# sea-with-sakura/ViT-of-Pytorch

Hardware: AMD Instinct MI355X
Metric: images/sec training step, ViT-B/16 224px bf16, 1/2/4/8 MI355X (higher is better)
Workload: dtype bf16; 1 GPU; ViT-B16 @224 train step (fwd+CE+bwd+SGD-momentum/OneCycleLR); model=ViT-B16, image_size=224, per_gpu_batch=256, global_batch=256, seq_len=197, num_classes=1000, parallelism=dp1, step_launch=eager

## Files before the change

vit-of-pytorch_amd/csrc/gemm.hip:

```cpp
#include "gemm_decl.h"

namespace {
using vitg::GemmDev;
using vitg::EPI_DROP;

int pick_tile(const vit_gemm_args* a) {
  if (a->tile > 0) return (int)a->tile;
  const bool ak = a->a_layout == VIT_K_CONTIG, bk = a->b_layout == VIT_K_CONTIG;
  if (a->epilogue == VIT_EPI_SPLITK && a->M >= 256 && a->N >= 256) {
    static const int env_sk = vit::knob("VIT_GEMM_SPLITK_CFG", 9);
    return env_sk == 5 || env_sk == 6 || env_sk == 7 || env_sk == 8 ? env_sk : 9;
  }
  if (a->M >= 1024 && a->N >= 256) {
    static const int env_rs = vit::knob("VIT_GEMM_RESID_PP2", 1);
    if (ak && (env_rs || !(a->epilogue == VIT_EPI_BIAS_RESID_F32 && a->K < 2048))) return 9;
    if (a->N >= 2048 && a->epilogue != VIT_EPI_GELU_BWD && a->epilogue != VIT_EPI_MUL_BF16) return 5;
    if (!bk && a->K >= 3072) return 5;
    return 3;
  }
  return 0;
}

int tile_rows_of(int cfg) {
  switch (cfg) {
    case 1: case 2: case 3: case 5: case 6: case 7: case 8: case 9: case 10: case 11: return 256;
    default: return 128;
  }
}

long wave_split_rows(const vit_gemm_args* a, int cfg) {
  if (!((cfg == 5 || cfg == 9) && a->batch == 1 && a->split_k == 1 && a->epilogue != VIT_EPI_PATCH && a->tile == 0))
    return 0;
  static const int ncu = [] {
    int dev = 0, n = 0;
    if (hipGetDevice(&dev) != hipSuccess || hipDeviceGetAttribute(&n, hipDeviceAttributeMultiprocessorCount, dev) !=
                                               hipSuccess)
      return 0;
    return n;
  }();
  if (ncu <= 0) return 0;
  const long tiles_n = (a->N + 255) / 256, tiles = ((a->M + 255) / 256) * tiles_n;
  const long full = tiles / ncu, rem = tiles - full * ncu;
  const long main_rows = (full * ncu / tiles_n) * 256;
  return full >= 1 && rem > 0 && 2 * rem <= ncu && main_rows > 0 && main_rows < a->M ? main_rows : 0;
}

int rem_config() {
  static const int rem_cfg = vit::knob("VIT_GEMM_REM_CFG", 0);
  return rem_cfg >= 0 && rem_cfg <= 9 && rem_cfg != 1 ? rem_cfg : 0;
}

}

extern "C" int64_t vit_gemm_tile_rows(const vit_gemm_args* a) {
  if (!a) return 0;
  return tile_rows_of(pick_tile(a));
}

extern "C" int64_t vit_gemm_partial_rows(const vit_gemm_args* a) {
  if (!a) return 0;
  const int cfg = pick_tile(a);
  const long main_rows = wave_split_rows(a, cfg);
  if (main_rows > 0) {
    const long rr = tile_rows_of(rem_config());
    return main_rows / 256 + (a->M - main_rows + rr - 1) / rr;
  }
  const long tr = tile_rows_of(cfg);
  return (a->M + tr - 1) / tr;
}

extern "C" int64_t vit_gemm_split_rows(const vit_gemm_args* a) {
  if (!a) return 0;
  return wave_split_rows(a, pick_tile(a));
}

#ifdef VIT_PP2_STAMPS
static unsigned long long* g_pp2_stamp_buf = nullptr;
extern "C" int vit_gemm_set_stamps(void* dev_buf) {
  g_pp2_stamp_buf = (unsigned long long*)dev_buf;
  return 0;
}
#endif

namespace {
int make_dev(const vit_gemm_args* a, GemmDev& d, bool& empty) {
  empty = false;
  VIT_CHECK_ARG(a != nullptr, "vit_gemm_bf16: null args");
  VIT_CHECK_ARG(a->M >= 0 && a->N >= 0 && a->K >= 0, "vit_gemm_bf16: negative size");
  VIT_CHECK_ARG(a->K % 64 == 0, "vit_gemm_bf16: K=%lld must be a multiple of 64", (long long)a->K);
  VIT_CHECK_ARG(a->M < (1 << 30) && a->N < (1 << 30), "vit_gemm_bf16: M/N too large");
  VIT_CHECK_ARG(a->A && a->B && a->C, "vit_gemm_bf16: null operand");
  VIT_CHECK_ARG(a->batch >= 1 && a->split_k >= 1, "vit_gemm_bf16: batch/split_k must be >= 1");
  VIT_CHECK_ARG(a->split_k == 1 || a->epilogue == VIT_EPI_SPLITK, "vit_gemm_bf16: split_k>1 needs VIT_EPI_SPLITK");
  VIT_CHECK_ARG(a->a_layout == VIT_K_CONTIG || a->a_layout == VIT_MN_CONTIG, "vit_gemm_bf16: bad a_layout");
  VIT_CHECK_ARG(a->b_layout == VIT_K_CONTIG || a->b_layout == VIT_MN_CONTIG, "vit_gemm_bf16: bad b_layout");
  if (a->M == 0 || a->N == 0) {
    empty = true;
    return VIT_OK;
  }
  const bool ak = a->a_layout == VIT_K_CONTIG, bk = a->b_layout == VIT_K_CONTIG;
  const long a_rows = ak ? a->M : a->K, a_cols = ak ? a->K : a->M;
  const long b_rows = bk ? a->N : a->K, b_cols = bk ? a->K : a->N;
  VIT_CHECK_ARG(a->lda >= a_cols && a->ldb >= b_cols, "vit_gemm_bf16: leading dimension too small");
  VIT_CHECK_ARG(a->lda % 8 == 0 && a->ldb % 8 == 0, "vit_gemm_bf16: lda/ldb must be multiples of 8");
  VIT_CHECK_ARG(((uintptr_t)a->A | (uintptr_t)a->B) % 16 == 0 && (a->a_batch_stride | a->b_batch_stride) % 8 == 0,
                "vit_gemm_bf16: A/B must be 16-byte aligned");
  const long a_bytes = ((a_rows - 1) * a->lda + ((a_cols + 7) & ~7L)) * 2;
  const long b_bytes = ((b_rows - 1) * a->ldb + ((b_cols + 7) & ~7L)) * 2;
  VIT_CHECK_ARG(a_bytes < (1L << 31) && b_bytes < (1L << 31), "vit_gemm_bf16: operand larger than 2 GiB");
  switch (a->epilogue) {
    case VIT_EPI_BIAS_GELU: VIT_CHECK_ARG(a->C2 != nullptr, "GELU epilogue needs C2"); break;
    case VIT_EPI_BIAS_RESID_F32: VIT_CHECK_ARG(a->aux != nullptr, "RESID epilogue needs aux"); break;
    case VIT_EPI_GELU_BWD: VIT_CHECK_ARG(a->aux != nullptr, "GELU_BWD epilogue needs aux"); break;
    case VIT_EPI_MUL_BF16: VIT_CHECK_ARG(a->aux != nullptr, "MUL epilogue needs aux"); break;
    case VIT_EPI_BIAS_GELU_DGELU: VIT_CHECK_ARG(a->C2 != nullptr, "GELU_DGELU epilogue needs C2"); break;
    case VIT_EPI_PATCH:
      VIT_CHECK_ARG(a->aux && a->aux2 && a->bias && a->tokens > 0 && a->batch == 1, "PATCH epilogue args");
      break;
    default: break;
  }
  d = GemmDev{};
  d.M = (int)a->M; d.N = (int)a->N; d.K = (int)a->K;
  d.A = (const char*)a->A; d.lda = a->lda; d.a_bs = a->a_batch_stride; d.a_bytes = (uint32_t)a_bytes;
  d.B = (const char*)a->B; d.ldb = a->ldb; d.b_bs = a->b_batch_stride; d.b_bytes = (uint32_t)b_bytes;
  d.C = a->C; d.ldc = a->ldc; d.c_bs = a->c_batch_stride;
  d.C2 = a->C2; d.ldc2 = a->ldc2;
  d.bias = a->bias; d.bias_bs = a->bias_batch_stride;
  d.aux = a->aux; d.ldaux = a->ldaux; d.aux2 = a->aux2;
  d.split_k = (int)a->split_k; d.tokens = (int)a->tokens;
  {
    auto al = [](const void* q) { return ((uintptr_t)q % 32) == 0; };
    bool v = al(a->C) && a->ldc % 8 == 0 && a->c_batch_stride % 8 == 0;
    if (a->C2) v = v && al(a->C2) && a->ldc2 % 8 == 0;
    if (a->bias) v = v && al(a->bias) && a->bias_batch_stride % 8 == 0;
    if (a->aux) v = v && al(a->aux) && a->ldaux % 8 == 0;
    if (a->aux2) v = v && al(a->aux2);
    if (a->epilogue == VIT_EPI_SPLITK) v = al(a->C) && a->N % 8 == 0;
    d.vec = v ? 1 : 0;
  }
  d.col_partial = a->col_partial;
  d.drop = make_drop(a->dropout);
  VIT_CHECK_ARG(!d.drop.thr || a->epilogue == VIT_EPI_PATCH || a->epilogue == VIT_EPI_BIAS_RESID_F32 ||
                    a->epilogue == VIT_EPI_BIAS_GELU_DGELU,
                "vit_gemm_bf16: dropout is supported on the PATCH, BIAS_RESID_F32 and BIAS_GELU_DGELU epilogues");
  VIT_CHECK_ARG(!d.drop.thr || (a->a_layout == VIT_K_CONTIG &&
                                  (a->b_layout == VIT_K_CONTIG || a->epilogue == VIT_EPI_BIAS_RESID_F32)),
                "vit_gemm_bf16: dropout epilogues need a K-contiguous A (and B, except BIAS_RESID_F32)");
  {
    static const int env_gm = vit::knob("VIT_GEMM_GROUP_M", 8);
    static const int env_nt = vit::knob("VIT_GEMM_NT", 0);
    d.group_m = env_gm;
    d.nt = env_nt;
    static const int env_diag = vit::knob("VIT_GEMM_DIAG", 0);
    d.diag = env_diag;
    static const int env_sx = vit::knob("VIT_GEMM_SPLIT_XCD", 1);
    d.split_xcd = env_sx;
    static const int env_prio = vit::knob("VIT_GEMM_PRIO", 1);
    d.prio = env_prio;
    static const int env_ilv = vit::knob("VIT_GEMM_ILV", -1);
    d.ilv = env_ilv;
#ifdef VIT_PP2_STAMPS
    d.stamps = g_pp2_stamp_buf;
#endif
  }
  return VIT_OK;
}

int gemm_bf16_impl(const vit_gemm_args* a, int part, vit_stream_t stream) {
  GemmDev d;
  bool empty = false;
  if (const int rc = make_dev(a, d, empty)) return rc;
  if (empty) return VIT_OK;
  const bool ak = a->a_layout == VIT_K_CONTIG, bk = a->b_layout == VIT_K_CONTIG;
  if (a->col_partial) {
    VIT_CHECK_ARG(a->batch == 1 && a->split_k == 1 && d.vec && a->N % 8 == 0 &&
                      (a->epilogue == VIT_EPI_F32 || a->epilogue == VIT_EPI_BF16 || a->epilogue == VIT_EPI_GELU_BWD ||
                       a->epilogue == VIT_EPI_MUL_BF16 ||
                       a->epilogue == VIT_EPI_BIAS_BF16 || a->epilogue == VIT_EPI_BIAS_RESID_F32),
                  "vit_gemm_bf16: col_partial needs batch 1, split_k 1, aligned N%%8==0 operands and a plain epilogue");
  }
  hipStream_t s = (hipStream_t)stream;
  const int batch = (int)a->batch, split = (int)a->split_k;
  const int cfg = pick_tile(a);
#ifdef VIT_DIAG_KNOBS
  VIT_CHECK_ARG(cfg >= 0 && cfg <= 11, "vit_gemm_bf16: bad tile config %d", cfg);
#else
  VIT_CHECK_ARG(cfg >= 0 && cfg <= 9, "vit_gemm_bf16: bad tile config %d", cfg);
#endif
  VIT_CHECK_ARG(cfg != 1 || a->K % 32 == 0, "vit_gemm_bf16: K");
  auto run = [&](int c, const GemmDev& g) -> hipError_t {
    switch (a->epilogue) {
      case VIT_EPI_F32: return vitg::launch_layout_x<VIT_EPI_F32>(c, g, ak, bk, batch, split, s);
      case VIT_EPI_BF16: return vitg::launch_layout_x<VIT_EPI_BF16>(c, g, ak, bk, batch, split, s);
      case VIT_EPI_BIAS_BF16: return vitg::launch_layout_x<VIT_EPI_BIAS_BF16>(c, g, ak, bk, batch, split, s);
      case VIT_EPI_BIAS_GELU: return vitg::launch_layout_x<VIT_EPI_BIAS_GELU>(c, g, ak, bk, batch, split, s);
      case VIT_EPI_BIAS_RESID_F32:
        if (g.drop.thr) return vitg::launch_kk_x<VIT_EPI_BIAS_RESID_F32 | EPI_DROP>(c, g, bk, batch, split, s);
        return vitg::launch_layout_x<VIT_EPI_BIAS_RESID_F32>(c, g, ak, bk, batch, split, s);
      case VIT_EPI_GELU_BWD: return vitg::launch_layout_x<VIT_EPI_GELU_BWD>(c, g, ak, bk, batch, split, s);
      case VIT_EPI_BIAS_GELU_DGELU:
        if (g.drop.thr) return vitg::launch_kk_x<VIT_EPI_BIAS_GELU_DGELU | EPI_DROP>(c, g, bk, batch, split, s);
        return vitg::launch_layout_x<VIT_EPI_BIAS_GELU_DGELU>(c, g, ak, bk, batch, split, s);
      case VIT_EPI_MUL_BF16: return vitg::launch_layout_x<VIT_EPI_MUL_BF16>(c, g, ak, bk, batch, split, s);
      case VIT_EPI_PATCH:
        if (g.drop.thr) return vitg::launch_kk_x<VIT_EPI_PATCH | EPI_DROP>(c, g, bk, batch, split, s);
        return vitg::launch_layout_x<VIT_EPI_PATCH>(c, g, ak, bk, batch, split, s);
      case VIT_EPI_SPLITK: return vitg::launch_layout_x<VIT_EPI_SPLITK>(c, g, ak, bk, batch, split, s);
      default: return hipErrorInvalidValue;
    }
  };
  if (a->epilogue < 0 || a->epilogue > VIT_EPI_MUL_BF16) {
    vit::set_error("vit_gemm_bf16: unknown epilogue %d", a->epilogue);
    return VIT_ERR_INVALID_ARG;
  }
  if (const long main_rows = wave_split_rows(a, cfg)) {
    GemmDev g1 = d, g2 = d;
    g1.M = (int)main_rows;
    g2.M = (int)(a->M - main_rows);
    const long r0 = main_rows;
    const long a_off = ak ? r0 * a->lda * 2 : r0 * 2;
    g2.A = d.A + a_off;
    g2.a_bytes = d.a_bytes > a_off ? (uint32_t)(d.a_bytes - a_off) : 0u;
    const int csz = (a->epilogue == VIT_EPI_F32 || a->epilogue == VIT_EPI_BIAS_RESID_F32) ? 4 : 2;
    g2.C = (char*)d.C + r0 * a->ldc * csz;
    if (d.C2) g2.C2 = (char*)d.C2 + r0 * a->ldc2 * 2;
    if (d.aux) g2.aux = (const char*)d.aux + r0 * a->ldaux * (a->epilogue == VIT_EPI_BIAS_RESID_F32 ? 4 : 2);
    if (d.col_partial) g2.col_partial = d.col_partial + (main_rows / 256) * a->N;
    g2.drop.row0 = (int)r0;
    hipError_t e = hipSuccess;
    if (part != 2) e = run(cfg, g1);
    if (e == hipSuccess && part != 1) e = run(rem_config(), g2);
    return vit::check_hip(e, "vit_gemm_bf16 launch");
  }
  if (part == 2) return VIT_OK;
  return vit::check_hip(run(cfg, d), "vit_gemm_bf16 launch");
}
}

extern "C" int vit_gemm_bf16(const vit_gemm_args* a, vit_stream_t stream) { return gemm_bf16_impl(a, 0, stream); }

extern "C" int vit_gemm_bf16_part(const vit_gemm_args* a, int32_t part, vit_stream_t stream) {
  VIT_CHECK_ARG(part == 1 || part == 2, "vit_gemm_bf16_part: part %d (1 = whole-wave rows, 2 = remainder)", part);
  return gemm_bf16_impl(a, part, stream);
}

extern "C" int vit_gemm_splitk_group(const vit_gemm_args* args, int32_t n, vit_stream_t stream) {
  VIT_CHECK_ARG(args != nullptr && n >= 1 && n <= vitg::GEMM_GROUP_MAX, "vit_gemm_splitk_group: 1..%d members, got %d",
                vitg::GEMM_GROUP_MAX, n);
  vitg::GemmGroup g{};
  long total = 0;
  for (int i = 0; i < n; ++i) {
    const vit_gemm_args* a = args + i;
    VIT_CHECK_ARG(a->epilogue == VIT_EPI_SPLITK && a->a_layout == VIT_MN_CONTIG && a->b_layout == VIT_MN_CONTIG &&
                      a->tile == 0 && !a->col_partial && !a->dropout,
                  "vit_gemm_splitk_group: member %d must be a split-K weight gradient (VIT_EPI_SPLITK, both operands "
                  "M/N-contiguous, no tile / col_partial / dropout)", i);
    bool empty = false;
    if (const int rc = make_dev(a, g.g[i], empty)) return rc;
    VIT_CHECK_ARG(!empty, "vit_gemm_splitk_group: member %d is empty", i);
    g.start[i] = (int)total;
    total += ((a->M + 255) / 256) * ((a->N + 255) / 256) * a->split_k * a->batch;
    VIT_CHECK_ARG(total < (1L << 30), "vit_gemm_splitk_group: grid too large");
  }
  g.start[n] = (int)total;
  g.n = n;
  return vit::check_hip(vitg::launch_splitk_group(g, (hipStream_t)stream), "vit_gemm_splitk_group launch");
}

namespace {
__global__ void splitk_reduce_kernel(const float* __restrict__ ws, int split, long M, long N, float* __restrict__ out,
                                     long ldo, long obs, int accumulate) {
  const int z = blockIdx.y;
  const long total = M * N;
  const float* w = ws + (long)z * split * total;
  float* o = out + z * obs;
  for (long i = (long)blockIdx.x * blockDim.x + threadIdx.x; i < total; i += (long)gridDim.x * blockDim.x) {
    float s = 0.f;
    for (int k = 0; k < split; ++k) s += w[k * total + i];
    const long m = i / N, n = i - m * N;
    float* dst = o + m * ldo + n;
    *dst = accumulate ? *dst + s : s;
  }
}
__global__ void splitk_reduce4_kernel(const float* __restrict__ ws, int split, long M, long N, float* __restrict__ out,
                                      long ldo, long obs, int accumulate) {
  const int z = blockIdx.y;
  const long total = M * N, total4 = total / 4;
  const float4* w = reinterpret_cast<const float4*>(ws + (long)z * split * total);
  float* o = out + z * obs;
  for (long i = (long)blockIdx.x * blockDim.x + threadIdx.x; i < total4; i += (long)gridDim.x * blockDim.x) {
    float4 s = make_float4(0.f, 0.f, 0.f, 0.f);
    int k = 0;
    for (; k + 4 <= split; k += 4) {
      const float4 a = w[(long)k * total4 + i], b = w[(long)(k + 1) * total4 + i];
      const float4 c = w[(long)(k + 2) * total4 + i], d = w[(long)(k + 3) * total4 + i];
      s.x += (a.x + b.x) + (c.x + d.x);
      s.y += (a.y + b.y) + (c.y + d.y);
      s.z += (a.z + b.z) + (c.z + d.z);
      s.w += (a.w + b.w) + (c.w + d.w);
    }
    for (; k < split; ++k) {
      const float4 a = w[(long)k * total4 + i];
      s.x += a.x; s.y += a.y; s.z += a.z; s.w += a.w;
    }
    const long e = i * 4, m = e / N, n = e - m * N;
    float4* dst = reinterpret_cast<float4*>(o + m * ldo + n);
    if (accumulate) {
      const float4 p = *dst;
      s.x += p.x; s.y += p.y; s.z += p.z; s.w += p.w;
    }
    *dst = s;
  }
}

struct SplitkJobDev {
  const float* ws;
  float* out;
  long M, N, ldo, obs;
  int split, batch, nb, blk0, acc;
};
struct SplitkGroupDev {
  SplitkJobDev j[VIT_SPLITK_GROUP_MAX];
  int n;
};
__global__ void splitk_reduce4_group_kernel(const SplitkGroupDev G) {
  int jx = 0;
#pragma unroll
  for (int k = 1; k < VIT_SPLITK_GROUP_MAX; ++k)
    if (k < G.n && (int)blockIdx.x >= G.j[k].blk0) jx = k;
  const SplitkJobDev& J = G.j[jx];
  const int local = blockIdx.x - J.blk0;
  const int z = local / J.nb, bx = local - z * J.nb;
  const long total = J.M * J.N, total4 = total / 4;
  const float4* w = reinterpret_cast<const float4*>(J.ws + (long)z * J.split * total);
  float* o = J.out + z * J.obs;
  for (long i = (long)bx * blockDim.x + threadIdx.x; i < total4; i += (long)J.nb * blockDim.x) {
    float4 s = make_float4(0.f, 0.f, 0.f, 0.f);
    int k = 0;
    for (; k + 4 <= J.split; k += 4) {
      const float4 a = w[(long)k * total4 + i], b = w[(long)(k + 1) * total4 + i];
      const float4 c = w[(long)(k + 2) * total4 + i], d = w[(long)(k + 3) * total4 + i];
      s.x += (a.x + b.x) + (c.x + d.x);
      s.y += (a.y + b.y) + (c.y + d.y);
      s.z += (a.z + b.z) + (c.z + d.z);
      s.w += (a.w + b.w) + (c.w + d.w);
    }
    for (; k < J.split; ++k) {
      const float4 a = w[(long)k * total4 + i];
      s.x += a.x; s.y += a.y; s.z += a.z; s.w += a.w;
    }
    const long e = i * 4, m = e / J.N, n = e - m * J.N;
    float4* dst = reinterpret_cast<float4*>(o + m * J.ldo + n);
    if (J.acc) {
      const float4 p = *dst;
      s.x += p.x; s.y += p.y; s.z += p.z; s.w += p.w;
    }
    *dst = s;
  }
}
}

extern "C" int vit_splitk_reduce_group(const vit_splitk_job* jobs, int32_t n, vit_stream_t stream) {
  VIT_CHECK_ARG(jobs && n >= 1 && n <= VIT_SPLITK_GROUP_MAX, "vit_splitk_reduce_group: 1..%d jobs, got %d",
                VIT_SPLITK_GROUP_MAX, (int)n);
  bool vec = true;
  for (int k = 0; k < n; ++k) {
    const vit_splitk_job& j = jobs[k];
    VIT_CHECK_ARG(j.ws && j.out && j.batch >= 1 && j.split >= 1 && j.M >= 1 && j.N >= 1 && j.ldo >= j.N,
                  "vit_splitk_reduce_group: job %d: bad args", k);
    vec = vec && j.N % 4 == 0 && j.ldo % 4 == 0 && j.out_batch_stride % 4 == 0 && ((uintptr_t)j.ws % 16) == 0 &&
          ((uintptr_t)j.out % 16) == 0;
  }
  if (!vec) {
    for (int k = 0; k < n; ++k) {
      const vit_splitk_job& j = jobs[k];
      if (const int rc = vit_splitk_reduce(j.ws, j.batch, j.split, j.M, j.N, j.out, j.ldo, j.out_batch_stride,
                                           j.accumulate, stream))
        return rc;
    }
    return VIT_OK;
  }
  SplitkGroupDev g{};
  long blk = 0;
  for (int k = 0; k < n; ++k) {
    const vit_splitk_job& j = jobs[k];
    long nb = (j.M * j.N / 4 + 255) / 256;
    if (nb > 4096) nb = 4096;
    SplitkJobDev& d = g.j[k];
    d.ws = j.ws; d.out = j.out; d.M = j.M; d.N = j.N; d.ldo = j.ldo; d.obs = j.out_batch_stride;
    d.split = (int)j.split; d.batch = (int)j.batch; d.nb = (int)nb; d.blk0 = (int)blk; d.acc = j.accumulate ? 1 : 0;
    blk += nb * j.batch;
  }
  g.n = n;
  VIT_CHECK_ARG(blk < (1L << 31), "vit_splitk_reduce_group: grid too large");
  hipLaunchKernelGGL(splitk_reduce4_group_kernel, dim3((unsigned)blk), dim3(256), 0, (hipStream_t)stream, g);
  VIT_LAUNCH_CHECK("vit_splitk_reduce_group");
}

extern "C" int vit_splitk_reduce(const float* ws, int64_t batch, int64_t split, int64_t M, int64_t N, float* out,
                                 int64_t ldo, int64_t out_batch_stride, int32_t accumulate, vit_stream_t stream) {
  VIT_CHECK_ARG(ws && out && batch >= 1 && split >= 1 && ldo >= N, "vit_splitk_reduce: bad args");
  if (M * N == 0) return VIT_OK;
  const bool vec = N % 4 == 0 && ldo % 4 == 0 && out_batch_stride % 4 == 0 && ((uintptr_t)ws % 16) == 0 &&
                   ((uintptr_t)out % 16) == 0;
  long blocks = (M * N / (vec ? 4 : 1) + 255) / 256;
  if (blocks > 4096) blocks = 4096;
  if (vec)
    hipLaunchKernelGGL(splitk_reduce4_kernel, dim3((unsigned)blocks, (unsigned)batch), dim3(256), 0,
                       (hipStream_t)stream, ws, (int)split, (long)M, (long)N, out, (long)ldo, (long)out_batch_stride,
                       (int)accumulate);
  else
    hipLaunchKernelGGL(splitk_reduce_kernel, dim3((unsigned)blocks, (unsigned)batch), dim3(256), 0, (hipStream_t)stream,
                       ws, (int)split, (long)M, (long)N, out, (long)ldo, (long)out_batch_stride, (int)accumulate);
  VIT_LAUNCH_CHECK("vit_splitk_reduce");
}
```

vit-of-pytorch_amd/csrc/gemm_decl.h:

```cpp
#pragma once
#include "common.h"
#include <stdlib.h>

namespace vitg {

struct GemmDev {
  int M, N, K;
  const char* A;
  long lda;
  long a_bs;
  uint32_t a_bytes;
  const char* B;
  long ldb;
  long b_bs;
  uint32_t b_bytes;
  void* C;
  long ldc;
  long c_bs;
  void* C2;
  long ldc2;
  const float* bias;
  long bias_bs;
  const void* aux;
  long ldaux;
  const float* aux2;
  int split_k;
  int tokens;
  int vec;
  float* col_partial;
  int group_m;
  int nt;
  DropDev drop;
  int diag;
  int split_xcd;
  int prio;
  int ilv;
#ifdef VIT_PP2_STAMPS
  unsigned long long* stamps;
#endif
};

constexpr int GEMM_GROUP_MAX = 4;
struct GemmGroup {
  GemmDev g[GEMM_GROUP_MAX];
  int start[GEMM_GROUP_MAX + 1];
  int n;
};
hipError_t launch_splitk_group(const GemmGroup& g, hipStream_t s);

constexpr int EPI_DROP = 16;

template <int EPI>
hipError_t launch_layout_x(int cfg, const GemmDev& d, bool ak, bool bk, int batch, int split, hipStream_t s);
template <int EPI>
hipError_t launch_kk_x(int cfg, const GemmDev& d, bool bk, int batch, int split, hipStream_t s);
template <> hipError_t launch_layout_x<0>(int, const GemmDev&, bool, bool, int, int, hipStream_t);
template <> hipError_t launch_layout_x<1>(int, const GemmDev&, bool, bool, int, int, hipStream_t);
template <> hipError_t launch_layout_x<2>(int, const GemmDev&, bool, bool, int, int, hipStream_t);
template <> hipError_t launch_layout_x<3>(int, const GemmDev&, bool, bool, int, int, hipStream_t);
template <> hipError_t launch_layout_x<4>(int, const GemmDev&, bool, bool, int, int, hipStream_t);
template <> hipError_t launch_layout_x<5>(int, const GemmDev&, bool, bool, int, int, hipStream_t);
template <> hipError_t launch_layout_x<6>(int, const GemmDev&, bool, bool, int, int, hipStream_t);
template <> hipError_t launch_layout_x<7>(int, const GemmDev&, bool, bool, int, int, hipStream_t);
template <> hipError_t launch_layout_x<8>(int, const GemmDev&, bool, bool, int, int, hipStream_t);
template <> hipError_t launch_layout_x<9>(int, const GemmDev&, bool, bool, int, int, hipStream_t);
template <> hipError_t launch_kk_x<20>(int, const GemmDev&, bool, int, int, hipStream_t);
template <> hipError_t launch_kk_x<22>(int, const GemmDev&, bool, int, int, hipStream_t);
template <> hipError_t launch_kk_x<24>(int, const GemmDev&, bool, int, int, hipStream_t);
}
```

vit-of-pytorch_amd/csrc/gemm_pp2.inc:

```
template <bool AK, bool BKC, int EPI, int BK = 64, int NA = 2>
__device__ __forceinline__ void pp2_tile(const GemmDev& p, const int tm, const int tn, const int z,
                                         const int split_idx, const int orig) {
  constexpr int BM = 256, BN = 256, KK = BK / 32;
  constexpr int NB = NA + 1;
  constexpr int TN = BN / 4, FM = 8, FN = TN / 16;
  constexpr int HALF = 128 * BK * 2;
  constexpr int A0_OFF = 0, A1_OFF = NA * HALF, B_OFF = 2 * NA * HALF;
  constexpr int LDS = (2 * NA + 2 * NB) * HALF;
  constexpr int I = BK / 16;
  constexpr int LDW = TN + 4;
  constexpr int PR = 32;
  constexpr int WST = PR * LDW * 4;
  static_assert(8 * WST <= LDS && LDS <= 160 * 1024, "LDS budget / epilogue staging");
  static_assert(2 * I * (NA - 1) <= 32 && (2 * NA - 1) * I <= 62 && 2 * (NB - 1) * I <= 62, "vmcnt range");
  __shared__ __attribute__((aligned(16))) char smem[LDS];

  const int lane = threadIdx.x & 63;
  const int wave = __builtin_amdgcn_readfirstlane(threadIdx.x >> 6);
  const int grp = wave >> 2, wn = wave & 3;
  const int m0 = tm * BM, n0 = tn * BN;
  if (p.diag >= 100 && ((orig >> 3) & 1) && (orig >> 3) < 32) {
    const unsigned long long t0 = __builtin_amdgcn_s_memrealtime();
    while (__builtin_amdgcn_s_memrealtime() - t0 < (unsigned long long)(p.diag - 100) * 100ull)
      __builtin_amdgcn_s_sleep(8);
  }

  const char* Ab = p.A + (long)z * p.a_bs * 2;
  const char* Bb = p.B + (long)z * p.b_bs * 2;
  const long a_shift = AK ? (long)m0 * p.lda * 2 : (long)m0 * 2;
  const long b_shift = BKC ? (long)n0 * p.ldb * 2 : (long)n0 * 2;
  const uint32_t a_rec = (long)p.a_bytes > a_shift ? (uint32_t)(p.a_bytes - a_shift) : 0u;
  const uint32_t b_rec = (long)p.b_bytes > b_shift ? (uint32_t)(p.b_bytes - b_shift) : 0u;
  const __amdgpu_buffer_rsrc_t rsA = make_rsrc(Ab + a_shift, a_rec);
  const __amdgpu_buffer_rsrc_t rsB = make_rsrc(Bb + b_shift, b_rec);
  const int a_h1 = AK ? (int)(128 * p.lda * 2) : 256;
  const int b_h1 = BKC ? (int)(128 * p.ldb * 2) : 256;

  const int nkt = p.K / BK;
  const int kt0 = (int)((long)nkt * split_idx / p.split_k);
  const int kt1 = (int)((long)nkt * (split_idx + 1) / p.split_k);
  const int nk = kt1 - kt0;

  v4f acc[FM][FN];
#pragma unroll
  for (int i = 0; i < FM; ++i)
#pragma unroll
    for (int j = 0; j < FN; ++j) acc[i][j] = v4f{0.f, 0.f, 0.f, 0.f};
  v8s af[KK][FM], bfr[KK][FN];
  const int w4 = wave & 3;
#ifdef VIT_PP2_STAMPS
  const bool stw = p.diag == 4 && p.stamps && orig == 0 && split_idx == 0 && z == 0 && w4 == 0;
  unsigned long long stv[8] = {0, 0, 0, 0, 0, 0, 0, 0};
#define PP2_ST(k)                                          \
  do {                                                     \
    if (stw && j == nk / 2) {                              \
      __builtin_amdgcn_sched_barrier(0);                   \
      stv[k] = __builtin_amdgcn_s_memtime();               \
      __builtin_amdgcn_sched_barrier(0);                   \
    }                                                      \
  } while (0)
#else
#define PP2_ST(k) \
  do {            \
  } while (0)
#endif

  auto ld_a = [&](int h, int t) {
    stage_tile<128, BK, AK, 4>(smem, (h ? A1_OFF : A0_OFF) + (t % NA) * HALF, rsA, p.lda, kt0 + t, w4, lane,
                               h ? a_h1 : 0);
  };
  auto ld_b = [&](int h, int t) {
    stage_tile<128, BK, BKC, 4>(smem, B_OFF + (t % NB) * 2 * HALF + h * HALF, rsB, p.ldb, kt0 + t, w4, lane,
                                h ? b_h1 : 0);
  };
  uint32_t a_lane[AK ? 1 : FM], b_lane[BKC ? 1 : FN];
  if constexpr (!AK) {
#pragma unroll
    for (int i = 0; i < FM; ++i) a_lane[i] = frag_tr_lane_off<128>(i * 16, lane);
  }
  if constexpr (!BKC) {
#pragma unroll
    for (int jn = 0; jn < FN; ++jn) b_lane[jn] = frag_tr_lane_off<128>((wn & 1) * 64 + jn * 16, lane);
  }
  const uint32_t s0 = (uint32_t)(uintptr_t)LDS_PTR(char, smem);
  auto mem = [&](int t) {
    const int aoff = (grp ? A1_OFF : A0_OFF) + (t % NA) * HALF;
    const int boff = B_OFF + (t % NB) * 2 * HALF + (wn >> 1) * HALF;
    const uint32_t ab = __builtin_amdgcn_readfirstlane(s0 + aoff), bb = __builtin_amdgcn_readfirstlane(s0 + boff);
#pragma unroll
    for (int kk = 0; kk < KK; ++kk) {
#pragma unroll
      for (int jn = 0; jn < FN; ++jn) {
        if constexpr (BKC)
          bfr[kk][jn] = read_frag<128, BK, BKC>(smem, boff, (wn & 1) * 64 + jn * 16, kk, lane);
        else
          bfr[kk][jn] = kk == 0 ? read_frag_tr_asm<128, 0>(b_lane[jn] + bb) : read_frag_tr_asm<128, 1>(b_lane[jn] + bb);
      }
#pragma unroll
      for (int i = 0; i < FM; ++i) {
        if constexpr (AK)
          af[kk][i] = read_frag<128, BK, AK>(smem, aoff, i * 16, kk, lane);
        else
          af[kk][i] = kk == 0 ? read_frag_tr_asm<128, 0>(a_lane[i] + ab) : read_frag_tr_asm<128, 1>(a_lane[i] + ab);
      }
    }
  };
#ifdef VIT_DIAG_KNOBS
  const bool ilv = p.ilv < 0 ? (!AK && !BKC) : p.ilv > 0;
#else
  constexpr bool ilv = !AK && !BKC;
#endif
  auto frag = [&](int t, int f) {
    constexpr int NF = FN + FM;
    const int kk = f / NF, r = f % NF;
    const int aoff = (grp ? A1_OFF : A0_OFF) + (t % NA) * HALF;
    const int boff = B_OFF + (t % NB) * 2 * HALF + (wn >> 1) * HALF;
    const uint32_t ab = __builtin_amdgcn_readfirstlane(s0 + aoff), bb = __builtin_amdgcn_readfirstlane(s0 + boff);
    if (r < FN) {
      if constexpr (BKC)
        bfr[kk][r] = read_frag<128, BK, BKC>(smem, boff, (wn & 1) * 64 + r * 16, kk, lane);
      else
        bfr[kk][r] = kk == 0 ? read_frag_tr_asm<128, 0>(b_lane[r] + bb) : read_frag_tr_asm<128, 1>(b_lane[r] + bb);
    } else {
      const int i = r - FN;
      if constexpr (AK)
        af[kk][i] = read_frag<128, BK, AK>(smem, aoff, i * 16, kk, lane);
      else
        af[kk][i] = kk == 0 ? read_frag_tr_asm<128, 0>(a_lane[i] + ab) : read_frag_tr_asm<128, 1>(a_lane[i] + ab);
    }
  };
  auto piece = [&](int q, int j, bool g1) {
    __builtin_amdgcn_sched_barrier(0);
    if (q < I) {
      const int t = g1 ? j + NA : j + NA - 1;
      if (t < nk)
        stage_piece<128, BK, AK, 4>(smem, (g1 ? A0_OFF : A1_OFF) + (t % NA) * HALF, rsA, p.lda, kt0 + t, w4, lane,
                                    g1 ? 0 : a_h1, q);
    } else {
      const int t = j + NB - 1;
      if (t < nk)
        stage_piece<128, BK, BKC, 4>(smem, B_OFF + (t % NB) * 2 * HALF + (g1 ? HALF : 0), rsB, p.ldb, kt0 + t, w4,
                                     lane, g1 ? b_h1 : 0, q - I);
    }
    __builtin_amdgcn_sched_barrier(0);
  };
  auto slot_ilv = [&](int j, bool g1) {
    constexpr int NFR = KK * (FN + FM), NP = 2 * I, PER = NFR / NP;
    static_assert(PER * NP == NFR, "whole fragments between pieces");
#pragma unroll
    for (int f = 0; f < NFR; ++f) {
      frag(j, f);
      if (f % PER == PER - 1) piece(f / PER, j, g1);
    }
  };
  auto reads_done = [&]() {
    asm volatile("s_waitcnt lgkmcnt(0)" ::: "memory");
    __builtin_amdgcn_sched_barrier(0);
  };
  auto compute = [&]() {
    if (p.prio == 1) __builtin_amdgcn_s_setprio(1);
#pragma unroll
    for (int kk = 0; kk < KK; ++kk)
#pragma unroll
      for (int i = 0; i < FM; ++i)
#pragma unroll
        for (int jn = 0; jn < FN; ++jn)
          acc[i][jn] = __builtin_amdgcn_mfma_f32_16x16x32_bf16(__builtin_bit_cast(v8bf, af[kk][i]),
                                                               __builtin_bit_cast(v8bf, bfr[kk][jn]), acc[i][jn], 0, 0, 0);
    if (p.prio == 1) __builtin_amdgcn_s_setprio(0);
  };
  auto read_prio = [&](bool hi) {
    if (p.prio == 2) {
      if (hi) __builtin_amdgcn_s_setprio(1);
      else __builtin_amdgcn_s_setprio(0);
    }
  };
  auto barrier = [&]() {
    __builtin_amdgcn_sched_barrier(0);
    asm volatile("s_barrier" ::: "memory");
    __builtin_amdgcn_sched_barrier(0);
  };
  auto wait_younger = [&](int younger) {
    __builtin_amdgcn_sched_barrier(0);
    if constexpr (NA == 2 && I == 4) {
      if (younger >= 8)
        wait_vm<8>();
      else if (younger >= 4)
        wait_vm<4>();
      else
        wait_vm<0>();
    } else {
      switch (younger / I) {
        case 0: wait_vm<0>(); break;
        case 1: wait_vm<I>(); break;
        case 2: wait_vm<2 * I>(); break;
        case 3: wait_vm<3 * I>(); break;
        case 4: wait_vm<4 * I>(); break;
        case 5: wait_vm<5 * I>(); break;
        case 6: wait_vm<6 * I>(); break;
        case 7: wait_vm<7 * I>(); break;
        default: wait_vm<8 * I>(); break;
      }
    }
  };
  auto dma0 = [&](int j) { return j < 0 ? 0 : I * ((j + NA - 1 < nk) + (j + NB - 1 < nk)); };
  auto dma1 = [&](int j) { return j < 0 ? 0 : I * ((j + NA < nk) + (j + NB - 1 < nk)); };
  auto in_flight = [&](int j, bool g1) {
    int n = 0;
#pragma unroll
    for (int d = 0; d < NA - 1; ++d) n += g1 ? dma1(j - d) : dma0(j - d);
    return n;
  };

  if (grp == 0) {
#pragma unroll
    for (int t = 0; t < NA; ++t)
      if (t < nk) ld_a(0, t);
#pragma unroll
    for (int t = 0; t < NA - 1; ++t)
      if (t < nk) ld_a(1, t);
  } else {
#pragma unroll
    for (int t = 0; t < NB - 1; ++t)
      if (t < nk) {
        ld_b(0, t);
        ld_b(1, t);
      }
  }
  wait_vm<0>();
  __builtin_amdgcn_s_barrier();
  asm volatile("" ::: "memory");

  if (grp == 0) {
    for (int j = 0; j < nk; ++j) {
      PP2_ST(0);
      read_prio(true);
      if (ilv) {
        slot_ilv(j, false);
        PP2_ST(1);
      } else {
        mem(j);
        PP2_ST(1);
        if (j + NA - 1 < nk) ld_a(1, j + NA - 1);
        if (j + NB - 1 < nk) ld_b(0, j + NB - 1);
      }
      read_prio(false);
      PP2_ST(2);
      reads_done();
      PP2_ST(3);
      wait_younger(in_flight(j, false));
      PP2_ST(4);
      barrier();
      PP2_ST(5);
      compute();
      PP2_ST(6);
      barrier();
      PP2_ST(7);
    }
  } else if (nk > 0) {
    barrier();
    for (int j = 0; j < nk; ++j) {
      PP2_ST(0);
      read_prio(true);
      if (ilv) {
        slot_ilv(j, true);
        PP2_ST(1);
      } else {
        mem(j);
        PP2_ST(1);
        if (j + NA < nk) ld_a(0, j + NA);
        if (j + NB - 1 < nk) ld_b(1, j + NB - 1);
      }
      read_prio(false);
      PP2_ST(2);
      reads_done();
      PP2_ST(3);
      wait_younger(in_flight(j, true));
      PP2_ST(4);
      barrier();
      PP2_ST(5);
      compute();
      PP2_ST(6);
      if (j + 1 < nk) barrier();
      PP2_ST(7);
    }
  }
#ifdef VIT_PP2_STAMPS
  if (stw && lane == 0) {
#pragma unroll
    for (int k = 0; k < 8; ++k) p.stamps[grp * 8 + k] = stv[k];
  }
#endif
#undef PP2_ST

  if (p.diag == 2) {
    float t = 0.f;
#pragma unroll
    for (int i = 0; i < FM; ++i)
#pragma unroll
      for (int jn = 0; jn < FN; ++jn) t += acc[i][jn][0] + acc[i][jn][1] + acc[i][jn][2] + acc[i][jn][3];
    if (t == 1234.5f) ((float*)p.C)[threadIdx.x] = t;
    return;
  }
  const int wm0 = grp * 128, wn0 = wn * TN;
  const int g = lane >> 4, c = lane & 15;
  float* ws = reinterpret_cast<float*>(smem + wave * WST);
  constexpr int CPR = TN / 8;
  float csum[8] = {0.f, 0.f, 0.f, 0.f, 0.f, 0.f, 0.f, 0.f};
  constexpr int IT = PR * CPR / 64;
  static_assert(IT * 64 == PR * CPR, "whole chunks per pass");
  constexpr int AW = AuxPre<EPI>::W > 0 ? AuxPre<EPI>::W : 1;
  uint4 axc[IT][AW], axn[IT][AW];
  auto fetch_pass = [&](uint4 (*ax)[AW], int pass) {
    if constexpr (AuxPre<EPI>::W > 0) {
#pragma unroll
      for (int it = 0; it < IT; ++it) {
        const int e = lane + it * 64, row = e / CPR, ch = e % CPR;
        const int m = m0 + wm0 + pass * PR + row, n = n0 + wn0 + ch * 8;
        if (p.vec && m < p.M && n + 8 <= p.N) AuxPre<EPI>::fetch(p, m, n, ax[it]);
      }
    }
  };
  if (EpiOut<EPI>::FAST && p.vec && p.diag == 0 && m0 + BM <= p.M && n0 + BN <= p.N) {
    epilogue_fast<EPI, FN, LDW, CPR>(p, acc, ws, lane, m0 + wm0, n0 + wn0, z, split_idx, csum);
  } else {
  fetch_pass(axc, 0);
#pragma unroll
  for (int pass = 0; pass < 128 / PR; ++pass) {
    if (pass + 1 < 128 / PR) fetch_pass(axn, pass + 1);
#pragma unroll
    for (int i = 0; i < PR / 16; ++i)
#pragma unroll
      for (int jn = 0; jn < FN; ++jn)
#pragma unroll
        for (int r = 0; r < 4; ++r) ws[(i * 16 + 4 * g + r) * LDW + jn * 16 + c] = acc[pass * (PR / 16) + i][jn][r];
    asm volatile("s_waitcnt lgkmcnt(0)" ::: "memory");
    __builtin_amdgcn_wave_barrier();
#pragma unroll
    for (int it = 0; it < IT; ++it) {
      const int e = lane + it * 64, row = e / CPR, ch = e % CPR;
      const int m = m0 + wm0 + pass * PR + row, n = n0 + wn0 + ch * 8;
      float v[8];
      ld8f(ws + row * LDW + ch * 8, v);
      if (m >= p.M || n >= p.N || p.diag == 1 || (p.diag == 3 && (blockIdx.x & 1))) continue;
      if (p.vec && n + 8 <= p.N) {
        if constexpr (AuxPre<EPI>::W > 0) {
          float u[8];
          AuxPre<EPI>::unpack(axc[it], u);
          epi_store8<EPI>(p, z, split_idx, m, n, v, u);
        } else {
          epi_store8<EPI>(p, z, split_idx, m, n, v);
        }
        if (p.col_partial) {
#pragma unroll
          for (int k = 0; k < 8; ++k) csum[k] += v[k];
        }
      } else {
#pragma unroll
        for (int k = 0; k < 8; ++k) epi_store<EPI>(p, z, split_idx, m, n + k, v[k]);
      }
    }
    asm volatile("s_waitcnt lgkmcnt(0)" ::: "memory");
    __builtin_amdgcn_wave_barrier();
    if constexpr (AuxPre<EPI>::W > 0) {
#pragma unroll
      for (int it = 0; it < IT; ++it)
#pragma unroll
        for (int w = 0; w < AW; ++w) axc[it][w] = axn[it][w];
    }
  }
  }
  if (p.col_partial) {
#pragma unroll
    for (int k = 0; k < 8; ++k)
#pragma unroll
      for (int o = CPR; o < 64; o <<= 1) csum[k] += __shfl_xor(csum[k], o, 64);
    __syncthreads();
    float* red = reinterpret_cast<float*>(smem);
    if (lane < CPR) {
#pragma unroll
      for (int k = 0; k < 8; ++k) red[grp * BN + wn0 + lane * 8 + k] = csum[k];
    }
    __syncthreads();
    for (int col = threadIdx.x; col < BN; col += 512)
      if (n0 + col < p.N) p.col_partial[(long)tm * p.N + n0 + col] = red[col] + red[BN + col];
  }
}

__device__ __forceinline__ void splitk_coords(const GemmDev& p, int w, int nwg, int tiles_m, int tiles_n, int& tm, int& tn,
                                              int& z, int& split_idx) {
  const int zs = w / nwg;
  z = zs / p.split_k;
  split_idx = zs % p.split_k;
  tile_coords(w % nwg, tiles_m, tiles_n, p.group_m, tm, tn);
}

__device__ __forceinline__ int xcd_major(int lin, int total) {
  const int xcd = lin & 7, q8 = total >> 3, r8 = total & 7;
  return (xcd < r8 ? xcd * (q8 + 1) : r8 * (q8 + 1) + (xcd - r8) * q8) + (lin >> 3);
}

template <bool AK, bool BKC, int EPI, int BK = 64, int NA = 2>
__global__ void __launch_bounds__(512) gemm_pp2_kernel(const GemmDev p) {
  const int tiles_m = (p.M + 255) / 256, tiles_n = (p.N + 255) / 256;
  const int nwg = tiles_m * tiles_n;
  const int orig = blockIdx.x;
  int tm, tn, z, split_idx;
  if (p.split_k > 1 && p.split_xcd) {
    const int total = nwg * p.split_k * (int)gridDim.z;
    const int lin = blockIdx.x + nwg * (blockIdx.y + p.split_k * blockIdx.z);
    splitk_coords(p, xcd_major(lin, total), nwg, tiles_m, tiles_n, tm, tn, z, split_idx);
  } else {
    tile_coords(xcd_major(orig, nwg), tiles_m, tiles_n, p.group_m, tm, tn);
    z = blockIdx.z;
    split_idx = blockIdx.y;
  }
  pp2_tile<AK, BKC, EPI, BK, NA>(p, tm, tn, z, split_idx, orig);
}

template <bool AK, bool BKC>
__global__ void __launch_bounds__(512) gemm_pp2_group_kernel(const GemmGroup G) {
  const int orig = blockIdx.x;
  const int w = xcd_major(orig, G.start[G.n]);
  int gi = 0;
#pragma unroll
  for (int k = 1; k < GEMM_GROUP_MAX; ++k)
    if (k < G.n && w >= G.start[k]) gi = k;
  gi = __builtin_amdgcn_readfirstlane(gi);
  const GemmDev& p = G.g[gi];
  const int tiles_m = (p.M + 255) / 256, tiles_n = (p.N + 255) / 256;
  int tm, tn, z, split_idx;
  splitk_coords(p, w - G.start[gi], tiles_m * tiles_n, tiles_m, tiles_n, tm, tn, z, split_idx);
  pp2_tile<AK, BKC, VIT_EPI_SPLITK>(p, tm, tn, z, split_idx, orig);
}

template <bool AK, bool BKC, int EPI, int BK = 64, int NA = 2>
hipError_t launch_pp2(const GemmDev& d, int batch, int split, hipStream_t s) {
  const int tiles = ((d.M + 255) / 256) * ((d.N + 255) / 256);
  dim3 grid(tiles, split, batch);
  hipLaunchKernelGGL((gemm_pp2_kernel<AK, BKC, EPI, BK, NA>), grid, dim3(512), 0, s, d);
  return hipGetLastError();
}

inline hipError_t launch_pp2_group(const GemmGroup& g, hipStream_t s) {
  hipLaunchKernelGGL((gemm_pp2_group_kernel<false, false>), dim3(g.start[g.n]), dim3(512), 0, s, g);
  return hipGetLastError();
}
```

Before: 7769 images/sec.

## Let each wave group load its own A half in the MN-contig pp2 GEMM

For the pp2 256x256 GEMM tile with both operands non-K-contiguous, each wave group now issues the global-to-LDS load of its own A half right after its compute phase. Before, the loads were spread across the two groups' interleaved fragment-read slots. The counted vmcnt waits are rewritten to match the new per-group in-flight load counts, and B loads stay interleaved with the fragment reads. The aim is to cut cross-group dependencies and put A prefetch under compute. The risk is a wrong wait count, which would race on LDS, and a different issue balance that can stall the memory pipe.

```diff
diff --git a/vit-of-pytorch_amd/csrc/gemm.hip b/vit-of-pytorch_amd/csrc/gemm.hip
--- a/vit-of-pytorch_amd/csrc/gemm.hip
+++ b/vit-of-pytorch_amd/csrc/gemm.hip
@@ -159,6 +159,8 @@
     d.prio = env_prio;
     static const int env_ilv = vit::knob("VIT_GEMM_ILV", -1);
     d.ilv = env_ilv;
+    static const int env_own = vit::knob("VIT_GEMM_OWN", 1);
+    d.own = env_own;
 #ifdef VIT_PP2_STAMPS
     d.stamps = g_pp2_stamp_buf;
 #endif
diff --git a/vit-of-pytorch_amd/csrc/gemm_decl.h b/vit-of-pytorch_amd/csrc/gemm_decl.h
--- a/vit-of-pytorch_amd/csrc/gemm_decl.h
+++ b/vit-of-pytorch_amd/csrc/gemm_decl.h
@@ -35,6 +35,7 @@
   int split_xcd;
   int prio;
   int ilv;
+  int own;
 #ifdef VIT_PP2_STAMPS
   unsigned long long* stamps;
 #endif
diff --git a/vit-of-pytorch_amd/csrc/gemm_pp2.inc b/vit-of-pytorch_amd/csrc/gemm_pp2.inc
--- a/vit-of-pytorch_amd/csrc/gemm_pp2.inc
+++ b/vit-of-pytorch_amd/csrc/gemm_pp2.inc
@@ -13,6 +13,8 @@
   constexpr int WST = PR * LDW * 4;
   static_assert(8 * WST <= LDS && LDS <= 160 * 1024, "LDS budget / epilogue staging");
   static_assert(2 * I * (NA - 1) <= 32 && (2 * NA - 1) * I <= 62 && 2 * (NB - 1) * I <= 62, "vmcnt range");
+  constexpr int OWN_PIECES = (!AK && !BKC && NA == 2) ? I : 0;
+  static_assert(OWN_PIECES == 0 || OWN_PIECES == I, "whole A halves move; the counted waits below assume it");
   __shared__ __attribute__((aligned(16))) char smem[LDS];
 
   const int lane = threadIdx.x & 63;
@@ -50,7 +52,7 @@
   const int w4 = wave & 3;
 #ifdef VIT_PP2_STAMPS
   const bool stw = p.diag == 4 && p.stamps && orig == 0 && split_idx == 0 && z == 0 && w4 == 0;
-  unsigned long long stv[8] = {0, 0, 0, 0, 0, 0, 0, 0};
+  unsigned long long stv[10] = {0, 0, 0, 0, 0, 0, 0, 0, 0, 0};
 #define PP2_ST(k)                                          \
   do {                                                     \
     if (stw && j == nk / 2) {                              \
@@ -106,8 +108,10 @@
     }
   };
 #ifdef VIT_DIAG_KNOBS
+  const bool own = OWN_PIECES > 0 && p.own != 0;
   const bool ilv = p.ilv < 0 ? (!AK && !BKC) : p.ilv > 0;
 #else
+  constexpr bool own = OWN_PIECES > 0;
   constexpr bool ilv = !AK && !BKC;
 #endif
   auto frag = [&](int t, int f) {
@@ -153,6 +157,20 @@
       if (f % PER == PER - 1) piece(f / PER, j, g1);
     }
   };
+  auto slot_ilv_own = [&](int j, bool g1) {
+    constexpr int NFR = KK * (FN + FM), PER = NFR / I;
+    static_assert(PER * I == NFR, "whole fragments between pieces");
+#pragma unroll
+    for (int f = 0; f < NFR; ++f) {
+      frag(j, f);
+      if (f % PER == PER - 1) piece(I + f / PER, j, g1);
+    }
+  };
+  auto own_half = [&](int t) {
+    __builtin_amdgcn_sched_barrier(0);
+    if (t < nk) ld_a(grp, t);
+    __builtin_amdgcn_sched_barrier(0);
+  };
   auto reads_done = [&]() {
     asm volatile("s_waitcnt lgkmcnt(0)" ::: "memory");
     __builtin_amdgcn_sched_barrier(0);
@@ -212,6 +230,10 @@
     return n;
   };
 
+  auto own_b = [&](int j) { return j < 0 ? 0 : I * (j + NB - 1 < nk); };
+  auto own_a0 = [&](int j) { return j < 0 ? 0 : I * (j + NA < nk); };
+  auto own_a1 = [&](int j) { return j < 0 ? 0 : I * (j + NA - 1 < nk); };
+
   if (grp == 0) {
 #pragma unroll
     for (int t = 0; t < NA; ++t)
@@ -235,7 +257,10 @@
     for (int j = 0; j < nk; ++j) {
       PP2_ST(0);
       read_prio(true);
-      if (ilv) {
+      if (own) {
+        slot_ilv_own(j, false);
+        PP2_ST(1);
+      } else if (ilv) {
         slot_ilv(j, false);
         PP2_ST(1);
       } else {
@@ -248,21 +273,34 @@
       PP2_ST(2);
       reads_done();
       PP2_ST(3);
-      wait_younger(in_flight(j, false));
+      wait_younger(own ? own_a0(j - 1) + own_b(j) : in_flight(j, false));
       PP2_ST(4);
       barrier();
       PP2_ST(5);
       compute();
       PP2_ST(6);
+      if (own) {
+        own_half(j + NA);
+        PP2_ST(7);
+        wait_younger(own_b(j) + own_a0(j));
+      }
+      PP2_ST(8);
       barrier();
-      PP2_ST(7);
+      PP2_ST(9);
     }
   } else if (nk > 0) {
+    if (own) {
+      own_half(NA - 1);
+      wait_younger(own_a1(0));
+    }
     barrier();
     for (int j = 0; j < nk; ++j) {
       PP2_ST(0);
       read_prio(true);
-      if (ilv) {
+      if (own) {
+        slot_ilv_own(j, true);
+        PP2_ST(1);
+      } else if (ilv) {
         slot_ilv(j, true);
         PP2_ST(1);
       } else {
@@ -275,20 +313,26 @@
       PP2_ST(2);
       reads_done();
       PP2_ST(3);
-      wait_younger(in_flight(j, true));
+      wait_younger(own ? own_a1(j) + own_b(j) : in_flight(j, true));
       PP2_ST(4);
       barrier();
       PP2_ST(5);
       compute();
       PP2_ST(6);
+      if (own && j + 1 < nk) {
+        own_half(j + NA);
+        PP2_ST(7);
+        wait_younger(own_b(j) + own_a1(j + 1));
+      }
+      PP2_ST(8);
       if (j + 1 < nk) barrier();
-      PP2_ST(7);
+      PP2_ST(9);
     }
   }
 #ifdef VIT_PP2_STAMPS
   if (stw && lane == 0) {
 #pragma unroll
-    for (int k = 0; k < 8; ++k) p.stamps[grp * 8 + k] = stv[k];
+    for (int k = 0; k < 10; ++k) p.stamps[grp * 10 + k] = stv[k];
   }
 #endif
 #undef PP2_ST
```

Result: no change. 7812 images/sec, median of 6 (+0.6%).
